# akloetgen/PARA-suite

Hardware: AMD Instinct MI355X
Metric: aligned reads/sec (10Mx50bp PAR-CLIP vs hg19-size genome) on MI355X; SAM bit-exact vs own CPU restatement (parity unpinned) (higher is better)
Workload: dtype u64

## Files before the change

### para-suite_amd/csrc/ps_kernels.hip

```cpp
#include <hip/hip_runtime.h>
#include <algorithm>
#include <cstdlib>
#include <stdexcept>
#include <string>
#include "ps_core.h"
#include "ps_narrow.h"
#include "ps_kernels.h"

namespace ps {

static const int PS_Q_CHUNK = 64;
#ifndef PS_BT_WAVES
#define PS_BT_WAVES 4
#endif

__device__ __forceinline__ unsigned long long wave_sum(unsigned long long v)
{
    for (int o = 32; o > 0; o >>= 1) v += __shfl_xor(v, o, 64);
    return v;
}
__device__ __forceinline__ void flush_stats(KStats *ks, const LaneStats &st)
{
    if (!ks) return;
    unsigned long long v[8] = {st.pairs, st.same, st.nodes, st.pushes, st.pops, st.lf, st.iters, st.exact};
// ... 100 lines not shown
        const unsigned long long wmask = __ballot(want), lmask = __ballot(L.mode != M_EXIT), hmask = __ballot(L.mode == M_HIT);
        if (lmask == 0) break;
        const bool stalled = (wmask | hmask) == lmask;
        const bool serve_hit = hmask != 0 && (__popcll(hmask) >= (int)hit_min || stalled);
        int fetch_r = -1;
        if (wmask) {
            const int cnt = __popcll(wmask);
            if (cnt >= (int)fetch_min || stalled) {
                const int rank = __popcll(wmask & lane_lt);
                int served = 0;
                while (served < cnt) {
                    if (q_next == q_end) {
                        if (exhausted) break;
                        unsigned int base = 0;
                        if (lane == 0) base = atomicAdd(queue, (unsigned int)PS_Q_CHUNK);
                        base = (unsigned int)__shfl((int)base, 0, 64);
                        if (base >= n_reads) { exhausted = true; break; }
                        q_next = (int)base;
                        q_end = (int)base + PS_Q_CHUNK < (int)n_reads ? (int)base + PS_Q_CHUNK : (int)n_reads;
                    }
                    const int take = q_end - q_next < cnt - served ? q_end - q_next : cnt - served;
                    if (want && rank >= served && rank < served + take) fetch_r = q_next + (rank - served);
                    q_next += take; served += take;
                }
                if (want && fetch_r < 0 && exhausted) fetch_r = (int)n_reads;
            }
        }
        bt_iter(a, h, L, m, fetch_r, serve_hit);
    }
    if (lane == 0) L.st.lf = (uint32_t)((wall_clock64() - t_start) >> 4);
    flush_stats(a.stats, L.st);
}


template <bool STATS, bool NB32>
__global__ void __launch_bounds__(256, PS_BT_WAVES) k_backtrack_n(const BtArgs *__restrict__ ap, BtHot hk, int lm_stride)
{
    const BtArgs &a = *ap;
    BtHot h; pin_hot(h, hk);
    uint32_t *const queue = reinterpret_cast<uint32_t *>(pin64(reinterpret_cast<unsigned long long>(a.queue)));
    const uint32_t n_reads = h.n_reads, fetch_min = pin32((uint32_t)a.fetch_min), hit_min = pin32((uint32_t)a.hit_min);
    extern __shared__ __attribute__((aligned(16))) uint8_t smem[];
    const int lane_g = blockIdx.x * blockDim.x + threadIdx.x;
    BtMem m;
    bt_mem_bind(m, smem + (size_t)threadIdx.x * lm_stride, h.len(), h.seed_len());
    uint8_t *const pool_private = reinterpret_cast<uint8_t *>(a.pool) + (size_t)lane_g * h.pool_cap * sizeof(Entry16);
    m.pool = pool_private;
    m.heads = nullptr;
    NLane L;
    nl_init(L);
    LaneStats st;
    ls_init(st);
    NtClock clk;
    for (int j = 0; j < 4; ++j) clk.tm[j] = 0;
    clk.t_last = 0;
#ifdef PS_STAMPS
    clk.t_last = __builtin_amdgcn_s_memtime();
#endif
    const int lane = threadIdx.x & 63;
    const unsigned long long t_start = STATS ? wall_clock64() : 0ull;
    uint32_t iters0 = 0;
    int q_next = 0, q_end = 0;
    bool exhausted = false;
    for (;;) {
        const int mode = nl_mode(L.ctl);
        const bool want = mode == M_FETCH;
        if (want && (L.ctl & NL_BIG)) {
            const unsigned int slot = (unsigned int)((reinterpret_cast<uint8_t *>(m.pool) - a.big_pool) / ((size_t)h.big_cap * sizeof(Entry16)));
            __threadfence();
            atomicExch(a.big_busy + slot, 0u);
            m.pool = pool_private;
            L.ctl &= ~NL_BIG;
        }
        const unsigned long long wmask = __ballot(want), lmask = __ballot(mode != M_EXIT), hmask = __ballot(mode == M_HIT);
        if (lmask == 0) break;
        const bool stalled = (wmask | hmask) == lmask;
        const bool serve_hit = hmask != 0 && (__popcll(hmask) >= (int)hit_min || stalled);
        int fetch_r = -1;
        if (wmask) {
            const int cnt = __popcll(wmask);
            if (cnt >= (int)fetch_min || stalled) {
                const int rank = (int)__builtin_amdgcn_mbcnt_hi((unsigned int)(wmask >> 32), __builtin_amdgcn_mbcnt_lo((unsigned int)wmask, 0u));
                int served = 0;
                while (served < cnt) {
                    if (q_next == q_end) {
                        if (exhausted) break;
                        unsigned int base = 0;
                        if (lane == 0) base = atomicAdd(queue, (unsigned int)PS_Q_CHUNK);
                        base = (unsigned int)__shfl((int)base, 0, 64);
                        if (base >= n_reads) { exhausted = true; break; }
                        q_next = (int)base;
                        q_end = (int)base + PS_Q_CHUNK < (int)n_reads ? (int)base + PS_Q_CHUNK : (int)n_reads;
                    }
                    const int take = q_end - q_next < cnt - served ? q_end - q_next : cnt - served;
                    if (want && rank >= served && rank < served + take) fetch_r = q_next + (rank - served);
                    q_next += take; served += take;
                }
                if (want && fetch_r < 0 && exhausted) fetch_r = (int)n_reads;
            }
        }
        unsigned long long gmask = __ballot(mode == M_GROW);
        while (gmask) {
            const int src = __ffsll((unsigned long long)gmask) - 1;
            gmask &= gmask - 1;
            const unsigned int n_big = a.n_big;
            unsigned int slot = n_big;
            if (lane == src) {
                unsigned int at = atomicAdd(a.big_next, 1u) % n_big;
                for (int tries = 0; tries < 256; ++tries) {
                    if (atomicCAS(a.big_busy + at, 0u, 1u) == 0u) { slot = at; break; }
                    at = at + 1u == n_big ? 0u : at + 1u;
                }
            }
            slot = (unsigned int)__shfl((int)slot, src, 64);
            const unsigned int n_copy = (unsigned int)__shfl((int)nl_bump(L), src, 64);
            const unsigned long long from = (unsigned long long)__shfl((long long)reinterpret_cast<unsigned long long>(m.pool), src, 64);
            if (slot < n_big) {
                const uint4 *sp = reinterpret_cast<const uint4 *>(from);
                uint4 *dp = reinterpret_cast<uint4 *>(a.big_pool + (size_t)slot * h.big_cap * sizeof(Entry16));
                for (unsigned int e = (unsigned int)lane; e < n_copy; e += 64u) dp[e] = sp[e];
                __threadfence();
                if (lane == src) { m.pool = dp; L.ctl = nl_set_mode(L.ctl | NL_BIG, M_EXPAND); }
            } else if (lane == src) L.ctl = nl_set_mode(nl_set_status(L.ctl, RS_OVERFLOW_POOL), M_POP);
        }
        nt_iter<STATS, NB32>(a, h, L, st, m, fetch_r, serve_hit, &clk);
        if (STATS && a.read_iters) {
            const int now = nl_mode(L.ctl);
            if (mode == M_FETCH && now != M_FETCH && now != M_EXIT) {
                iters0 = st.iters - 1u;
                const int len = nl_len(L), sl = h.seed_len();
                a.read_iters[PS_RI_WORDS * (size_t)L.r + 2] = (uint32_t)(m.cw[len - 1] & 0x7f) | ((h.use_seed() && sl > 0 && sl < len ? (uint32_t)(m.csw[sl - 1] & 0x7f) : 0u) << 8) | (a.est_ab ? (uint32_t)a.est_ab[L.r] << 16 : 0u);
                const uint32_t *cw32 = reinterpret_cast<const uint32_t *>(m.cw);
                for (int p = 0; p < 16; ++p) a.read_iters[PS_RI_WORDS * (size_t)L.r + 4 + p] = p < lm_ncw(len) ? cw32[p] : 0u;
            }
            if (mode != M_FETCH && mode != M_EXIT && now == M_FETCH) {
                uint32_t *ri = a.read_iters + PS_RI_WORDS * (size_t)L.r;
                ri[0] = st.iters - iters0; ri[1] = nl_bump(L);
                ri[3] = (uint32_t)nl_best_score(L) | ((uint32_t)nl_max_units(L) << 8) | ((uint32_t)nl_n_aln(L.ctl) << 16);
            }
        }
    }
    if (STATS) {
        if (lane == 0) st.lf = (uint32_t)((wall_clock64() - t_start) >> 4);
#ifdef PS_STAMPS
        st.nodes = lane == 0 ? (uint32_t)(clk.tm[0] >> 6) : 0; st.pushes = lane == 0 ? (uint32_t)(clk.tm[1] >> 6) : 0;
        st.pops = lane == 0 ? (uint32_t)(clk.tm[2] >> 6) : 0; st.exact = lane == 0 ? (uint32_t)(clk.tm[3] >> 6) : 0;
#endif
        flush_stats(a.stats, st);
    } else {
        st.nodes = st.pushes = st.pops = st.iters = st.exact = st.lf = 0;
        flush_stats(a.stats, st);
    }
}

__global__ void __launch_bounds__(256) k_sa2pos(IndexView ix, const bwtint *rows, bwtint *out, int n, KStats *stats)
{
    const int stride = gridDim.x * blockDim.x;
    int item = blockIdx.x * blockDim.x + threadIdx.x;
    LaneStats st = {0, 0, 0, 0, 0, 0, 0, 0};
    bool have = false; bwtint row = 0; uint32_t steps = 0;
    while (true) {
        if (!have) {
            if (item >= n) break;
            row = rows[item]; steps = 0; have = true;
        }
        if (!sa_walk_step(ix, row, steps, st)) {
            out[item] = (bwtint)steps + sa_sample(ix, row / (bwtint)ix.sa_intv);
            item += stride; have = false;
        }
    }
    flush_stats(stats, st);
}

__device__ __forceinline__ int text_sym(const IndexView &ix, bwtint p) { return p < ix.l_pac ? pac_base(ix.pac, p) : 3 - pac_base(ix.pac, 2 * ix.l_pac - 1 - p); }
__global__ void __launch_bounds__(256) k_index_check(IndexView ix, unsigned long long *out)
{
    unsigned long long rows = 0, bad_sym = 0, bad_sa = 0, longest = 0;
    const bwtint n_sa = ix.n_sa;
    for (bwtint t = (bwtint)blockIdx.x * blockDim.x + threadIdx.x; t < n_sa; t += (bwtint)gridDim.x * blockDim.x) {
        bwtint row = t * (bwtint)ix.sa_intv;
        bwtint p = t == 0 ? ix.seq_len : sa_sample(ix, t);
        unsigned long long steps = 0;
        do {
            if (p == 0) {
                if (row != ix.primary) ++bad_sym;
                row = 0; p = ix.seq_len;
            } else {
                if (row == ix.primary) { ++bad_sym; break; }
                int pos = 0;
                const uint32_t b = blk_of(row_to_stored(ix.primary, row), pos);
                Blk x;
                load_blk(ix.blocks, b, x);
                const int c = blk_sym(x, pos);
                if (c != text_sym(ix, p - 1)) ++bad_sym;
                row = L2_of(ix, c) + blk_count1(x, pos + 1, c);
                --p;
            }
// ... 23 lines not shown
    int32_t *E = H + (size_t)(a.len + 2) * 64;
    uint8_t *z = a.zbuf + (size_t)blockIdx.x * a.z_per_block + threadIdx.x;
    for (int it = blockIdx.x * 64 + threadIdx.x; it < a.n_items; it += gridDim.x * 64) {
        RefineItem q = a.items[it];
        const int qlen = a.lens ? a.lens[q.read] : a.len;
        int tlen = qlen + q.ref_shift;
        int d = tlen - qlen; if (d < 0) d = -d;
        int w = (int)(d * 1.5); if (w < 50) w = 50;
        const int r = q.read, len = qlen, n_reads = a.n_reads;
        const uint32_t *bases = a.bases, *nmask = a.nmask;
        const int strand = q.strand;
        uint32_t cig[PS_MAX_CIGAR];
        int n = banded_global(len,
            [&](int j) { int b = read_base(bases, nmask, n_reads, r, strand ? len - 1 - j : j); return b > 3 ? 4 : (strand ? 3 - b : b); },
            tlen, a.ix.pac, q.rb, w, H, E, 64, z, 64, cig, PS_MAX_CIGAR);
        a.n_cigar[it] = n;
        for (int j = 0; j < PS_MAX_CIGAR; ++j) a.cigar[(size_t)it * PS_MAX_CIGAR + j] = j < n ? cig[j] : 0;
    }
}

void launch_width(const WidthArgs &a, hipStream_t s)
{
    int blocks = (a.n_reads + 255) / 256;
    if (blocks > 256 * 8) blocks = 256 * 8;
    if (blocks < 1) blocks = 1;
    hipLaunchKernelGGL(k_width, dim3(a.use_seed ? 2 * blocks : blocks), dim3(256), 0, s, a);
}
__global__ void __launch_bounds__(256) k_jump_level(BtHot h, uint32_t *table, bwtint seq_len, int d)
{
    const uint32_t n = 1u << (2 * d);
    for (uint32_t s = blockIdx.x * blockDim.x + threadIdx.x; s < n; s += gridDim.x * blockDim.x) jump_fill_slot(h, table, seq_len, d, s);
}
void launch_jump_build(const IndexView &ix, uint32_t *table, int levels, hipStream_t s)
{
    BtArgs a{};
    a.ix = ix; a.ix.jump = nullptr; a.ix.jump_levels = 0;
    BtHot h;
    (void)bt_hot_make(a, h);
    for (int d = 0; d < levels; ++d) {
        const uint32_t n = 1u << (2 * d);
        const int blocks = (int)std::min<uint32_t>((n + 255u) / 256u, 256u * 16u);
        hipLaunchKernelGGL(k_jump_level, dim3(blocks), dim3(256), 0, s, h, table, ix.seq_len, d);
    }
}
bool launch_backtrack(const BtArgs &a_in, const BtArgs *d_args, BtArgs *h_stage, int n_blocks, int lm_stride, hipStream_t s, bool stats)
{
    BtArgs &a = *h_stage;
    a = a_in;
    const char *ej = std::getenv("PS_JUMP");
    const bool stats_plain = stats && !std::getenv("PS_STATS_JUMP");
    if (stats_plain || a.wide || (ej && std::atoi(ej) == 0)) { a.ix.jump = nullptr; a.ix.jump_levels = 0; }
    BtHot h;
    if (!bt_hot_make(a, h)) return false;
    (void)hipMemcpyAsync(const_cast<BtArgs *>(d_args), &a, sizeof(BtArgs), hipMemcpyHostToDevice, s);
    const size_t lds = (size_t)256 * lm_stride;
    const bool nb32 = a.md.n_buckets <= 32;
    typedef void (*KernelN)(const BtArgs *, BtHot, int);
    const KernelN kn = stats ? (nb32 ? k_backtrack_n<true, true> : k_backtrack_n<true, false>) : (nb32 ? k_backtrack_n<false, true> : k_backtrack_n<false, false>);
    const void *fn = a.wide ? reinterpret_cast<const void *>(k_backtrack_wide) : reinterpret_cast<const void *>(kn);
    set_dynamic_lds(fn, a.wide ? "k_backtrack_wide" : "k_backtrack_n", lds);
    if (a.wide) hipLaunchKernelGGL(k_backtrack_wide, dim3(n_blocks), dim3(256), lds, s, d_args, h, lm_stride);
    else hipLaunchKernelGGL(kn, dim3(n_blocks), dim3(256), lds, s, d_args, h, lm_stride);
    return true;
}
void launch_sa2pos(const IndexView &ix, const bwtint *rows, bwtint *out, int n, KStats *stats, hipStream_t s)
{
    int blocks = (n + 255) / 256;
    if (blocks > 256 * 8) blocks = 256 * 8;
    if (blocks < 1) blocks = 1;
    hipLaunchKernelGGL(k_sa2pos, dim3(blocks), dim3(256), 0, s, ix, rows, out, n, stats);
}
void launch_refine(const RefineArgs &a, int n_blocks, hipStream_t s)
{
    if (!a.hebuf || a.he_per_block < refine_he_words(a.len)) throw std::runtime_error("k_refine: H/E scratch missing or too small");
    hipLaunchKernelGGL(k_refine, dim3(n_blocks), dim3(64), 0, s, a);
}
void set_dynamic_lds(const void *kernel, const char *name, size_t bytes)
{
    if (bytes <= 48 * 1024) return;
    const std::string what = std::string(name) + ": " + std::to_string(bytes) + " B of dynamic LDS";
    if (bytes > PS_LDS_PER_CU) throw std::runtime_error(what + " requested, a CU has " + std::to_string(PS_LDS_PER_CU));
    const hipError_t e = hipFuncSetAttribute(kernel, hipFuncAttributeMaxDynamicSharedMemorySize, (int)bytes);
    if (e != hipSuccess) throw std::runtime_error(what + " refused: " + hipGetErrorString(e));
}

}
```

### para-suite_amd/csrc/ps_narrow.h

```cpp
#pragma once
#include "ps_core.h"

namespace ps {

PS_HD int nw_i(uint32_t wa) { return (int)(wa & 0xffu); }
PS_HD int nw_ldp(uint32_t wa) { return (int)((wa >> 8) & 0xffu); }
PS_HD int nw_mm(uint32_t wa) { return (int)((wa >> 16) & 0xffu); }
PS_HD int nw_state(uint32_t wa) { return (int)((wa >> 24) & 3u); }
PS_HD int nw_gapo(uint32_t wa) { return (int)((wa >> 26) & 7u); }
PS_HD int nw_gape(uint32_t wa) { return (int)(wa >> 29); }
PS_HD int nw_ins(uint32_t wb) { return (int)(wb & 7u); }
PS_HD int nw_del(uint32_t wb) { return (int)((wb >> 3) & 7u); }
PS_HD uint32_t nw_c(uint32_t wb) { return (wb >> 6) & 7u; }
PS_HD int nw_score(uint32_t wb) { return (int)((wb >> 9) & 0x7fu); }
static const uint32_t NW_KEEP = 0xFCFF0000u;
static const uint32_t NW_C_MASK = 7u << 6;
static const uint32_t NW_ROOT_C = 4u;

PS_HD int nl_mode(uint32_t ctl) { return (int)(ctl & 7u); }
PS_HD uint32_t nl_set_mode(uint32_t ctl, int mode) { return (ctl & ~7u) | (uint32_t)mode; }
static const uint32_t NL_HAVE_CUR = 8u, NL_STATUS = 7u << 4, NL_BIG = 1u << 7;
PS_HD int nl_status(uint32_t ctl) { return (int)((ctl >> 4) & 7u); }
PS_HD uint32_t nl_set_status(uint32_t ctl, int s) { return (ctl & ~NL_STATUS) | ((uint32_t)s << 4); }
PS_HD int nl_n_aln(uint32_t ctl) { return (int)(ctl >> 16); }

struct NLane {
    uint32_t kr, lr, wa, wb;
    uint32_t ctl;
    int r;
    uint32_t lim;
    uint32_t nsb;
    uint32_t n_phantom;
    uint32_t fh;
    uint32_t bm0, bm1;
    uint32_t rn0, rn1;
};
PS_HD int nl_best_score(const NLane &L) { return (int)(L.lim & 0xffu); }
PS_HD int nl_max_units(const NLane &L) { return (int)((L.lim >> 8) & 0xffu); }
PS_HD int nl_len(const NLane &L) { return (int)((L.lim >> 16) & 0xffu); }
PS_HD int nl_n_stack(const NLane &L) { return (int)(L.nsb & 0xffffu); }
PS_HD uint32_t nl_bump(const NLane &L) { return L.nsb >> 16; }
PS_HD uint32_t nl_phantom(const NLane &L) { return L.n_phantom & 0x00FFFFFFu; }
PS_HD int nl_est(const NLane &L) { return (int)(L.n_phantom >> 24); }

PS_HD void nl_init(NLane &L)
{
    L.kr = L.lr = L.wa = L.wb = 0; L.ctl = (uint32_t)M_FETCH; L.r = 0; L.lim = 0; L.nsb = 0;
    L.n_phantom = 0; L.fh = 0xffffu; L.bm0 = L.bm1 = 0; L.rn0 = L.rn1 = 0;
}
PS_HD void ls_init(LaneStats &st) { st.pairs = st.same = st.nodes = st.pushes = st.pops = st.iters = st.exact = st.lf = 0; }
PS_HD uint32_t ps_mul24(uint32_t x, uint32_t y)
{
#ifdef __HIP_DEVICE_COMPILE__
    return __umul24(x, y);
#else
    return x * y;
#endif
}

struct NtClock { unsigned long long tm[4]; unsigned long long t_last; };
#if defined(PS_STAMPS) && defined(__HIP_DEVICE_COMPILE__)
#define PS_USTAMP(clk, slot) do { if (STATS && (clk)) { const unsigned long long t_ = __builtin_amdgcn_s_memtime(); (clk)->tm[slot] += t_ - (clk)->t_last; (clk)->t_last = t_; } } while (0)
#else
#define PS_USTAMP(clk, slot) do { } while (0)
#endif

PS_HD bwtint nt_base(const BtHot &h, uint32_t c)
{
    return (bwtint)sel4s(h.L2lo[0], h.L2lo[1], h.L2lo[2], h.L2lo[3], (int)c) | ((bwtint)((h.L2hi >> c) & 1u) << 32);
}
PS_HD int nt_units(const BtHot &h, uint32_t wa, uint32_t wb)
{
    return h.profile() ? nw_score(wb) : nw_mm(wa) + nw_gapo(wa) + (h.mode_gape() ? nw_gape(wa) : 0);
}

PS_HD void blk_count4b(const Blk &b, int r, uint32_t cnt[4])
{
    uint32_t A = 0, B = 0, C = 0;
    const int q = r >> 5;
    const uint32_t part = (1u << (r & 31)) - 1u;
#pragma unroll
    for (int j = 0; j < 6; ++j) {
        const uint32_t m = j < q ? 0xFFFFFFFFu : (j == q ? part : 0u), lo = b.x[4 + j] & m, hi = b.x[10 + j] & m;
        A += ps_popc(lo); B += ps_popc(hi); C += ps_popc(lo & hi);
    }
    cnt[0] = b.x[0] + ((uint32_t)r - A - B + C);
    cnt[1] = b.x[1] + (A - C); cnt[2] = b.x[2] + (B - C); cnt[3] = b.x[3] + C;
}

#ifndef PS_OCC_COND
#define PS_OCC_COND 1
#endif
template <bool STATS>
PS_HD void nt_occ(const BtHot &h, uint32_t c, uint32_t kr, uint32_t lr, uint32_t ck[4], uint32_t cl[4], LaneStats &st)
{
    const bwtint base = nt_base(h, c);
    const bool need_k = c != NW_ROOT_C;
    int ol_ = 0, ok_ = 0;
    const uint32_t bl = blk_of(row_to_stored(h.primary, base + lr), ol_);
    uint32_t bk = blk_of(row_to_stored(h.primary, base + (bwtint)(need_k ? kr - 1u : 0u)), ok_);
    bk = need_k ? bk : 0u;
    const int rk = need_k ? ok_ + 1 : 0;
    Blk xl, xk;
    load_blk(h.blocks, bl, xl);
    if (PS_OCC_COND) {
        const bool other = bk != bl;
        if (other) load_blk(h.blocks, bk, xk);
        blk_count4b(xl, ol_ + 1, cl);
#pragma unroll
        for (int j = 0; j < 16; ++j) xk.x[j] = other ? xk.x[j] : xl.x[j];
    } else { load_blk(h.blocks, bk, xk); blk_count4b(xl, ol_ + 1, cl); }
    blk_count4b(xk, rk, ck);
    ++st.pairs; if (need_k && bk == bl) ++st.same;
// ... 218 lines not shown
        mode = M_POP;
    }
    if (mode == M_POP) {
        const int n_virtual = nl_n_stack(L) + ((L.ctl & NL_HAVE_CUR) ? 1 : 0);
        if (nl_phantom(L) && (long long)n_virtual + (long long)nl_phantom(L) > (long long)h.max_entries) {
            L.ctl = nl_set_status(L.ctl, RS_OVERFLOW_POOL); nt_finish_read(a, L); return 0;
        }
        if (n_virtual == 0 && nl_est(L) != 255 && nl_n_aln(L.ctl) == 0 && nl_status(L.ctl) == RS_OK) { NLane t = L; nt_restart_without_estimate(a, t, m); L = t; return 0; }
        if (n_virtual == 0 || n_virtual > (int)h.max_entries || nl_status(L.ctl) != RS_OK) { nt_finish_read(a, L); return 0; }
        if (L.ctl & NL_HAVE_CUR) L.ctl &= ~NL_HAVE_CUR;
        else { nt_pop<NB32>(L, m); if (STATS) ++st.pops; }
        L.ctl = nl_set_mode(L.ctl, M_POP);
        const int score = nw_score(L.wb), i1 = nw_i(L.wa);
        if (score > nl_best_score(L) + h.s_stop()) { nt_finish_read(a, L); return 0; }
        const int rem = nl_max_units(L) - nt_units(h, L.wa, L.wb);
        if (rem < 0) return 0;
        const int mleft = (int)(ps_mul24((uint32_t)rem, h.inv_c_min) >> 16);
        if (i1 > 0 && mleft < (int)(m.cw[i1 - 1] & 0x7f)) return 0;
        if (i1 == 0) { L.ctl = nl_set_mode(L.ctl, M_HIT); return 0; }
        const int st_ = nw_state(L.wa);
        mode = (mleft == 0 && (st_ == ST_M || h.mode_gape() || nw_gape(L.wa) == h.max_gape())) ? M_EXACT : M_EXPAND;
    }
    return mode;
}

struct NtStep { uint32_t ck[4], cl[4]; uint32_t cw_i, cw_im1, cs_i, cs_im1; int s, i; bool in_seed, tm, ctm; };

template <bool STATS>
PS_HD void nt_step_occ(const BtHot &h, NLane &L, LaneStats &st, BtMem &m, NtStep &q)
{
    const int len = nl_len(L), max_len = h.len();
    const int i = nw_i(L.wa) - 1;
    q.i = i;
    q.cw_i = m.cw[i]; q.cw_im1 = m.cw[i > 0 ? i - 1 : 0];
    const int ii = i - (len - h.seed_len());
    q.in_seed = h.use_seed() && len > h.seed_len() && ii > 0;
    q.cs_i = q.in_seed ? m.csw[ii] : 0u; q.cs_im1 = q.in_seed ? m.csw[ii - 1] : 0u;
    q.s = nt_seq_at(m, L, i, len, max_len);
    const int depth = nt_depth(len, L.wa, L.wb);
    q.tm = depth < (int)h.jump_levels; q.ctm = depth + 1 < (int)h.jump_levels;
    if (!q.tm) nt_occ<STATS>(h, nw_c(L.wb), L.kr, L.lr, q.ck, q.cl, st);
    else nt_jump(h, depth, L.kr, q.ck, q.cl);
}

template <bool STATS, bool NB32>
PS_HD void nt_tail(const BtHot &h, NLane &L, LaneStats &st, BtMem &m, const NtStep &q, int mode)
{
    const int len = nl_len(L), i = q.i, s = q.s;
    const uint32_t cw_i = q.cw_i, cw_im1 = q.cw_im1, cs_i = q.cs_i, cs_im1 = q.cs_im1;
    const bool in_seed = q.in_seed, tm = q.tm, ctm = q.ctm;
    uint32_t ck[4], cl[4];
#pragma unroll
    for (int c = 0; c < 4; ++c) { ck[c] = q.ck[c]; cl[c] = q.cl[c]; }
    if (mode == M_EXACT) {
        if (STATS) ++st.exact;
        L.ctl = nl_set_mode(L.ctl, M_POP);
        if (s > 3) return;
        const uint32_t ok = sel4(ck, s), ol = sel4(cl, s);
        if (ok >= ol) return;
        L.kr = ctm ? (L.kr << 2) | (uint32_t)s : ok + 1u; L.lr = ctm ? ol - ok : ol; L.wa -= 1u; L.wb = (L.wb & ~NW_C_MASK) | ((uint32_t)s << 6);
        L.ctl = nl_set_mode(L.ctl, i == 0 ? M_HIT : M_EXACT);
        return;
    }
    if (STATS) ++st.nodes;
    const uint32_t cap = (L.ctl & NL_BIG) ? h.big_cap : h.pool_cap;
    if (nl_bump(L) + 9u > cap) {
        if (!(L.ctl & NL_BIG) && h.has_big()) { L.ctl = nl_set_mode(L.ctl, M_GROW); return; }
        L.ctl = nl_set_mode(nl_set_status(L.ctl, cap >= 65535u ? RS_OVERFLOW_DEEP : RS_OVERFLOW_POOL), M_POP); return;
    }
    const int max_units = nl_max_units(L);
    const int e_un = nt_units(h, L.wa, L.wb), e_sc = nw_score(L.wb);
    const int rem = max_units - e_un;
    const uint32_t inv = h.inv_c_min;
    const int mleft = (int)(ps_mul24((uint32_t)rem, inv) >> 16);
    const int srem = h.seed_units() - e_un;
    const int m_seed = srem <= 0 ? 0 : (int)(ps_mul24((uint32_t)srem, inv) >> 16);
    bool allow_diff = true, allow_M = true;
    const int bnd_same = i > 0 ? (int)(cw_im1 & 0x7f) : 0;
    const int bnd_del = (int)(cw_i & 0x7f);
    if (i > 0) {
        if (bnd_same > mleft - 1) allow_diff = false;
        else if (bnd_same == mleft - 1 && bnd_del == mleft - 1 && (cw_i & 0x80u)) allow_M = false;
        if (in_seed) {
            const int s1 = (int)(cs_im1 & 0x7f), s0 = (int)(cs_i & 0x7f);
            if (s1 > m_seed - 1) allow_diff = false;
            else if (s1 == m_seed - 1 && s0 == m_seed - 1 && (cs_i & 0x80u)) allow_M = false;
        }
    }
    const int e_go = nw_gapo(L.wa), e_ge = nw_gape(L.wa), e_st = nw_state(L.wa);
    const int tmp = e_go + e_ge;
    const bool gap_ok = allow_diff && i >= h.indel_end_skip() + tmp && len - i >= h.indel_end_skip() + tmp;
    const bool from_m = e_st == ST_M, from_i = e_st == ST_I, from_d = e_st == ST_D;
    const uint32_t wa_keep = L.wa & NW_KEEP, pos2 = (uint32_t)i | ((uint32_t)i << 8);
    const uint32_t wb0 = L.wb & 0x1ffu;
    const uint32_t pkr = L.kr, plr = L.lr;
    const int need_same = (int)ps_mul24((uint32_t)bnd_same, h.c_min), need_del = (int)ps_mul24((uint32_t)bnd_del, h.c_min);
    const int cap_rem = nl_est(L) - e_sc, ut = h.u_tight();
    const int cap_same = cap_rem + (ut > need_same ? ut - need_same : 0), cap_del = cap_rem + (ut > need_del ? ut - need_del : 0);
    const int thr_same = (rem - need_same) < cap_same ? (rem - need_same) : cap_same, thr_del = (rem - need_del) < cap_del ? (rem - need_del) : cap_del;
    uint32_t phantom = 0, gmask = 0;
    int sc[9];
    uint32_t wa_i, wa_d;
    {
        const bool open = from_m && e_go < h.max_gapo(), ext = from_i && e_ge < h.max_gape();
        const int c = open ? h.u_gapo_ins() : h.u_gape();
        sc[0] = e_sc + (open ? h.s_gapo_ins() : h.s_gape());
        const bool cand = gap_ok && (open || ext) && c <= rem, go = cand && c <= thr_same;
        gmask |= go ? 1u : 0u;
        phantom += (cand && !go) ? 1u : 0u;
        wa_i = wa_keep + pos2 + ((uint32_t)ST_I << 24) + (open ? 1u << 26 : 1u << 29);
    }
    {
        const uint32_t occ = tm ? plr : plr - pkr + 1u;
        const bool open = from_m && e_go < h.max_gapo();
        const bool ext = from_d && e_ge < h.max_gape() && ((e_ge + e_go) * h.u_tight() < max_units || occ < (uint32_t)h.max_del_occ());
        const int c = open ? h.u_gapo_del() : h.u_gape();
        const int scd = e_sc + (open ? h.s_gapo_del() : h.s_gape());
        const bool cand = gap_ok && (open || ext) && c <= rem, go = cand && c <= thr_del;
        const uint32_t ne = (ck[0] < cl[0] ? 2u : 0u) | (ck[1] < cl[1] ? 4u : 0u) | (ck[2] < cl[2] ? 8u : 0u) | (ck[3] < cl[3] ? 16u : 0u);
        gmask |= go ? ne : 0u;
        if (cand && !go) phantom += ps_popc(ne);
        sc[1] = sc[2] = sc[3] = sc[4] = scd;
        wa_d = wa_keep + ((uint32_t)(i + 1) | ((uint32_t)(i + 1) << 8)) + ((uint32_t)ST_D << 24) + (open ? 1u << 26 : 1u << 29);
    }
    const bool do_mm = allow_diff && allow_M;
    const uint32_t s_word = cost_word(h.s_pk, s), u_word = h.profile() ? s_word : cost_word(h.u_pk, s);
    uint32_t xk[4], xl[4];
#pragma unroll
    for (int j = 1; j <= 4; ++j) {
        const int c = (s + j) & 3;
        xk[j - 1] = sel4(ck, c); xl[j - 1] = sel4(cl, c);
        sc[4 + j] = 0;
        if (j < 4 || s > 3) {
            const int cu = (int)((u_word >> (8 * c)) & 0xffu);
            sc[4 + j] = e_sc + (int)((s_word >> (8 * c)) & 0xffu);
            const bool cand = do_mm && xk[j - 1] < xl[j - 1] && cu <= rem, go = cand && cu <= thr_same;
            gmask |= go ? 1u << (4 + j) : 0u;
            phantom += (cand && !go) ? 1u : 0u;
        }
    }
    const uint32_t n_push = ps_popc(gmask), fr = L.fh;
    const bool reuse = fr != 0xffffu && n_push != 0u;
    const uint32_t slot0 = (L.nsb >> 16) - (reuse ? 1u : 0u);
    L.nsb += n_push + ((n_push - (reuse ? 1u : 0u)) << 16);
    L.fh = n_push ? 0xffffu : fr;
    if (STATS) st.pushes += n_push;
    uint32_t idx[9], raw[9];
#pragma unroll
    for (int j = 0; j < 9; ++j) {
        idx[j] = 0; raw[j] = 0;
        if ((gmask >> j) & 1u) {
            const uint32_t rank = ps_popc(gmask & ((1u << j) - 1u));
            idx[j] = (reuse && rank == 0u) ? fr : slot0 + rank;
            raw[j] = m.heads16[sc[j]];
            m.heads16[sc[j]] = (uint16_t)idx[j];
            if (NB32 || sc[j] < 32) L.bm0 |= 1u << sc[j]; else L.bm1 |= 1u << (sc[j] - 32);
        }
    }
#ifdef __HIP_DEVICE_COMPILE__
    asm volatile("" : "+v"(raw[0]), "+v"(raw[1]), "+v"(raw[2]), "+v"(raw[3]), "+v"(raw[4]), "+v"(raw[5]), "+v"(raw[6]), "+v"(raw[7]), "+v"(raw[8]));
#endif
    Entry16 *const pool = reinterpret_cast<Entry16 *>(m.pool);
#define NT_NEXT(j) (raw[j] << 16)
    if (gmask & 1u) { Entry16 e; e.k = pkr; e.l = plr; e.a = wa_i; e.b = (wb0 + 1u) | ((uint32_t)sc[0] << 9) | NT_NEXT(0); store16(pool + idx[0], e); }
    {
        const uint32_t wb_d = ((wb0 & 0x3fu) + (1u << 3)) | ((uint32_t)sc[1] << 9);
#pragma unroll
        for (int c = 0; c < 4; ++c)
            if ((gmask >> (1 + c)) & 1u) { Entry16 e; e.k = ctm ? (pkr << 2) | (uint32_t)c : ck[c] + 1u; e.l = ctm ? cl[c] - ck[c] : cl[c]; e.a = wa_d; e.b = wb_d | ((uint32_t)c << 6) | NT_NEXT(1 + c); store16(pool + idx[1 + c], e); }
    }
    {
        const uint32_t wa_x = wa_keep + pos2 + (1u << 16), wb_x = wb0 & 0x3fu;
#pragma unroll
        for (int j = 1; j <= 4; ++j) {
            const uint32_t c = (uint32_t)((s + j) & 3);
            if ((gmask >> (4 + j)) & 1u) { Entry16 e; e.k = ctm ? (pkr << 2) | c : xk[j - 1] + 1u; e.l = ctm ? xl[j - 1] - xk[j - 1] : xl[j - 1]; e.a = wa_x; e.b = wb_x | (c << 6) | ((uint32_t)sc[4 + j] << 9) | NT_NEXT(4 + j); store16(pool + idx[4 + j], e); }
        }
    }
#undef NT_NEXT
    L.ctl = nl_set_mode(L.ctl, M_POP);
    if (s < 4 && xk[3] < xl[3]) {
        L.kr = ctm ? (pkr << 2) | (uint32_t)s : xk[3] + 1u; L.lr = ctm ? xl[3] - xk[3] : xl[3]; L.wa = wa_keep + (uint32_t)i; L.wb = (L.wb & ~NW_C_MASK) | ((uint32_t)s << 6);
        L.ctl |= NL_HAVE_CUR;
    }
    L.n_phantom += phantom;
}

template <bool STATS, bool NB32>
PS_HD void nt_iter(const BtArgs &a, const BtHot &h, NLane &L, LaneStats &st, BtMem &m, int fetch_r, bool serve_hit, NtClock *clk = nullptr)
{
    PS_USTAMP(clk, 0);
    const int mode = nt_head<STATS, NB32>(a, h, L, st, m, fetch_r, serve_hit);
    PS_USTAMP(clk, 1);
    NtStep q;
    if (mode) nt_step_occ<STATS>(h, L, st, m, q);
#if defined(PS_STAMPS) && defined(__HIP_DEVICE_COMPILE__)
    if (STATS && clk && mode) asm volatile("" :: "v"(q.ck[0]), "v"(q.cl[0]), "v"(q.ck[3]), "v"(q.cl[3]));
#endif
    PS_USTAMP(clk, 2);
    if (mode) nt_tail<STATS, NB32>(h, L, st, m, q, mode);
    PS_USTAMP(clk, 3);
}

}
```

### para-suite_amd/csrc/ps_pipeline.hip

```cpp
#include <hip/hip_runtime.h>
#include <mutex>
#include <optional>
#include <hipcub/hipcub.hpp>
#include <algorithm>
#include <atomic>
#include <chrono>
#include <cmath>
#include <cstdio>
#include <cstring>
#include <functional>
#include <thread>
#include "ps_pipeline.h"
#include "ps_par.h"
#include "ps_core.h"

namespace ps {

typedef std::chrono::steady_clock Clock;
static double ms_since(Clock::time_point t0) { return std::chrono::duration<double, std::milli>(Clock::now() - t0).count(); }

void require_device(int device)
{
    int n = 0;
    hipError_t e = hipGetDeviceCount(&n);
// ... 319 lines not shown
                if (const char *e = std::getenv("PS_ORDER_SCALE")) em.log_scale = std::max(1, std::min(12, std::atoi(e)));
                if (d_lens) {
                    uint8_t *tab = wk->pin_get<uint8_t>("units_by_len_h2", 256);
                    for (int l2 = 0; l2 < 256; ++l2) { const int u = budget_diffs(ctx->opt, l2) * (ctx->opt.profile ? ctx->opt.unit : 1); tab[l2] = (uint8_t)(u > 255 ? 255 : u); }
                    uint8_t *d_tab = wk->ws_get<uint8_t>("units_by_len2", 256);
                    PS_HIP(hipMemcpyAsync(d_tab, tab, 256, hipMemcpyHostToDevice, s));
                    em.units_by_len = d_tab;
                }
                em.key = key; em.pred = nullptr;
                launch_effort_model(em, s);
            }
            launch_order_sort(key, n, wk->ws_get<uint32_t>("order_tmp", order_sort_tmp_words(n)), order, s);
            PS_HIP(hipGetLastError());
            t_order->mark();
            d_order = order; d_est = est;
        }
    }
    int dev_cus = 256;
    { hipDeviceProp_t p; if (hipGetDeviceProperties(&p, ctx->device) == hipSuccess && p.multiProcessorCount > 0) dev_cus = p.multiProcessorCount; }
    const int lm = lm_bytes(len, seed_len, md.n_buckets, wide);
    int per_cu = (int)((size_t)(160 * 1024) / ((size_t)256 * lm));
    if (per_cu < 1) throw Error("read length / score range too large for the per-lane LDS state");
    { const char *e = std::getenv("PS_MAX_PER_CU"); const int cap = e ? std::atoi(e) : 4; if (per_cu > cap) per_cu = cap; }
    int blocks = ctx->bt_blocks > 0 ? ctx->bt_blocks : dev_cus * per_cu;
    int need = (n + 255) / 256;
    if (blocks > need) blocks = need;
    const size_t per_lane = (size_t)pool_cap * (wide ? sizeof(Entry) : 16) + (wide ? PS_MAX_BUCKETS * 4 : 0);
    const size_t max_lanes = ((size_t)(wide ? 32 : 64) << 30) / per_lane;
    if ((size_t)blocks * 256 > max_lanes) blocks = (int)std::max<size_t>(1, max_lanes / 256);
    const int n_lanes = blocks * 256;
    uint8_t *pool = wk->ws_get<uint8_t>("pool", (size_t)n_lanes * pool_cap * (wide ? sizeof(Entry) : 16));
    uint32_t *heads = wide ? wk->ws_get<uint32_t>("heads", (size_t)n_lanes * PS_MAX_BUCKETS) : nullptr;
    uint32_t *queue = wk->ws_get<uint32_t>("queue", 16);
    PS_HIP(hipMemsetAsync(queue, 0, 64, s));
    BtArgs a; std::memset(&a, 0, sizeof a);
    a.ix = ctx->ix.view; a.md = md; a.n_reads = n; a.len = len; a.lens = d_lens; a.n_lanes = n_lanes;
    if (d_lens) {
        uint8_t *tab = wk->pin_get<uint8_t>("units_by_len_h", 256);
        for (int l2 = 0; l2 < 256; ++l2) { const int u = budget_diffs(ctx->opt, l2) * (ctx->opt.profile ? ctx->opt.unit : 1); tab[l2] = (uint8_t)(u > 255 ? 255 : u); }
        uint8_t *d_tab = wk->ws_get<uint8_t>("units_by_len", 256);
        PS_HIP(hipMemcpyAsync(d_tab, tab, 256, hipMemcpyHostToDevice, s));
        a.units_by_len = d_tab;
    }
    a.bases = d_bases; a.nmask = d_nmask; a.n_bw = (len + 15) / 16; a.n_mw = (len + 31) / 32;
    a.w = w; a.cwb = cwb; a.cswb = cswb;
    a.alns = alns; a.aln_cap = aln_cap; a.n_aln = n_aln; a.status = status;
    a.pool = pool; a.pool_cap = pool_cap; a.heads = heads; a.wide = wide ? 1 : 0; a.stats = b.d_stats.p + 1;
    a.queue = queue; a.fetch_min = ctx->fetch_min; a.hit_min = ctx->hit_min;
    a.order = d_order; a.est = d_est; a.est_ab = d_est_ab;
    a.cap_est = (first_tier && !wide && d_est && md.profile && !(std::getenv("PS_CAP") && std::atoi(std::getenv("PS_CAP")) == 0)) ? 1 : 0;
    if (a.cap_est) if (const char *e = std::getenv("PS_CAP_BIAS")) a.cap_est += std::max(0, std::min(200, std::atoi(e)));
    if (const char *e = std::getenv("PS_FETCH_MIN")) a.fetch_min = std::max(1, std::atoi(e));
    if (const char *e = std::getenv("PS_HIT_MIN")) a.hit_min = std::max(1, std::atoi(e));
    if (!wide && pool_cap < 65535 && ctx->n_big > 0) {
        a.big_cap = 65535; a.n_big = (uint32_t)std::min<int64_t>(ctx->n_big, std::max(64, n));
        a.big_pool = wk->ws_get<uint8_t>("big_pool", (size_t)a.n_big * a.big_cap * 16);
        a.big_next = queue + 4;
        a.big_busy = wk->ws_get<uint32_t>("big_busy", a.n_big);
        PS_HIP(hipMemsetAsync(a.big_busy, 0, (size_t)a.n_big * 4, s));
    }
    uint32_t *riters = nullptr;
    if (ctx->want_read_iters) { riters = wk->ws_get<uint32_t>("riters", (size_t)n * PS_RI_WORDS); PS_HIP(hipMemsetAsync(riters, 0, (size_t)n * PS_RI_WORDS * 4, s)); a.read_iters = riters; }
    { EvTimer t(s);
      if (!launch_backtrack(a, wk->ws_get<BtArgs>("btargs", 1), wk->pin_get<BtArgs>("btargs_h", 1), blocks, lm, s, ctx->want_kstats || ctx->want_read_iters)) throw Error("cost model outside the ranges the search kernel packs (gap/score fields must fit a byte)");
      PS_HIP(hipGetLastError());
      const double ms = t.stop(); b.tm.ms_backtrack += ms; ++b.tm.n_backtrack_launches;
      b.tm.ms_width += t_width->read();
      if (t_order) b.tm.ms_width += t_order->read();
      { double t0_ = 0, t1_ = 0; t.span(ctx->ref_event, t0_, t1_); if (b.tm.n_backtrack_launches == 1) b.tm.bt_begin_ms = t0_; b.tm.bt_end_ms = t1_; }
      if (std::getenv("PS_VERBOSE")) std::fprintf(stderr, "[parasuite-hip]   backtrack launch: %d reads x %d bp, stack %u%s, %d lanes, %.1f ms\n", n, len, pool_cap, wide ? " (wide)" : "", n_lanes, ms); }
    if (ctx->want_read_iters) { ctx->read_iters.resize((size_t)n * PS_RI_WORDS); PS_HIP(hipMemcpyAsync(ctx->read_iters.data(), riters, (size_t)n * PS_RI_WORDS * 4, hipMemcpyDeviceToHost, s)); PS_HIP(hipStreamSynchronize(s)); }
}

static void download_alns(Work *wk, int n, int aln_cap, const AlnRec *d_alns, const int32_t *d_n_aln,
                          std::vector<int32_t> &n_aln, std::vector<uint32_t> &off, std::vector<AlnRec> &alns)
{
    hipStream_t s = wk->stream;
    uint32_t *cnt = wk->ws_get<uint32_t>("cnt", n), *d_off = wk->ws_get<uint32_t>("off", (size_t)n + 1);
    hipLaunchKernelGGL(k_clip_counts, dim3((n + 255) / 256), dim3(256), 0, s, d_n_aln, aln_cap, n, cnt);
    size_t tb = 0;
    PS_HIP(hipcub::DeviceScan::ExclusiveSum(nullptr, tb, cnt, d_off, n, s));
    uint8_t *tmp = wk->ws_get<uint8_t>("scan_tmp", tb ? tb : 1);
    PS_HIP(hipcub::DeviceScan::ExclusiveSum(tmp, tb, cnt, d_off, n, s));
    int32_t *p_na = wk->pin_get<int32_t>("dl_n_aln", n); uint32_t *p_off = wk->pin_get<uint32_t>("dl_off", (size_t)n + 1);
    PS_HIP(hipMemcpyAsync(p_na, d_n_aln, (size_t)n * 4, hipMemcpyDeviceToHost, s));
    PS_HIP(hipMemcpyAsync(p_off, d_off, (size_t)n * 4, hipMemcpyDeviceToHost, s));
    PS_HIP(hipStreamSynchronize(s));
    uint32_t last = 0;
    if (n) { int m = p_na[n - 1]; last = p_off[n - 1] + (uint32_t)(m > aln_cap ? aln_cap : (m < 0 ? 0 : m)); }
    p_off[n] = last;
    n_aln.assign(p_na, p_na + n); off.assign(p_off, p_off + n + 1); alns.resize(last);
    if (last) {
        AlnRec *comp = wk->ws_get<AlnRec>("comp", last);
        hipLaunchKernelGGL(k_gather_alns, dim3((n + 255) / 256), dim3(256), 0, s, d_alns, aln_cap, d_n_aln, d_off, n, comp);
        AlnRec *p_al = wk->pin_get<AlnRec>("dl_alns", last);
        PS_HIP(hipMemcpyAsync(p_al, comp, (size_t)last * sizeof(AlnRec), hipMemcpyDeviceToHost, s));
        PS_HIP(hipStreamSynchronize(s));
        std::memcpy(alns.data(), p_al, (size_t)last * sizeof(AlnRec));
    }
}

__global__ void k_classify(const AlnRec *alns, int aln_cap, const int32_t *n_aln, const uint8_t *status, const int32_t *ids,
                           int n, int n_occ, uint8_t *cls_out)
{
    for (int r = blockIdx.x * blockDim.x + threadIdx.x; r < n; r += gridDim.x * blockDim.x) {
        uint8_t c = 0;
// ... 639 lines not shown
```

### para-suite_amd/csrc/ps_types.h

```cpp
#pragma once
#include <stdint.h>
#include <stddef.h>

#ifdef __HIPCC__
#define PS_HD __host__ __device__ __forceinline__
#define PS_COLD __host__ __device__ inline __attribute__((noinline))
#else
#define PS_HD inline
#define PS_COLD inline
#endif

namespace ps {

typedef uint64_t bwtint;
static const bwtint PS_MAX_ROWS = (1ull << 33) - 64;

static const int PS_BLK_SYMS = 192;
struct OccBlock { uint32_t cnt[4]; uint32_t sym[12]; };

struct IndexView {
    const OccBlock *blocks;
    const uint32_t *sa;
    const uint32_t *sa_hi;
    const uint8_t  *pac;
// ... 11 lines not shown
    uint8_t u_mm[5][4], s_mm[5][4];
    uint32_t u_mm_pk[5], s_mm_pk[5];
    int32_t u_gapo_ins, s_gapo_ins, u_gapo_del, s_gapo_del, u_gape, s_gape;
    int32_t s_stop, u_tight, c_min, inv_c_min , max_units, n_buckets;
    int32_t max_gapo, max_gape, mode_gape, indel_end_skip, max_del_occ, max_entries;
    int32_t seed_len, max_seed_diff, max_top2, use_seed, len, profile;
};
static const int PS_MAX_BUCKETS = 128;
static const int PS_MAX_LEN = 250;

struct Entry {
    bwtint k, l;
    uint16_t score, units;
    uint8_t i, last_diff_pos, n_mm, n_gapo, n_gape, n_ins, n_del, state;
    uint32_t next;
};
static const uint32_t PS_NIL = 0xFFFFFFFFu;
enum { ST_M = 0, ST_I = 1, ST_D = 2 };

struct AlnRec {
    bwtint k, l;
    uint16_t score, units;
    uint8_t n_mm, n_gapo, n_gape, n_ins, n_del, pad[7];
};

enum { RS_OK = 0, RS_OVERFLOW_POOL = 1, RS_OVERFLOW_ALN = 2, RS_BAD_SCORE = 3,
       RS_OVERFLOW_DEEP = 4 };

struct KStats {
    unsigned long long occ_pairs, occ_same_blk, nodes, pushes, pops, lf_steps, iters, exact_steps;
};

static const int PS_RI_WORDS = 20;
struct BtArgs {
    IndexView ix;
    Model md;
    int n_reads, len, n_lanes;
    const int32_t *lens;
    const uint8_t *units_by_len;
    const uint32_t *bases; const uint32_t *nmask; int n_bw, n_mw;
    uint32_t *w; const uint32_t *cwb; const uint32_t *cswb;
    AlnRec *alns; int aln_cap; int32_t *n_aln; uint8_t *status;
    void *pool; uint32_t pool_cap;
    uint32_t *heads;
    int wide;
    uint8_t *big_pool; uint32_t big_cap, n_big; uint32_t *big_busy; uint32_t *big_next;
    uint32_t *queue;
    const int32_t *order;
    const uint8_t *est; const uint16_t *est_ab;
    int cap_est;
    uint32_t *read_iters;
    int hit_min;
    int fetch_min;
    KStats *stats;
};

}
```

Measured before the change: 9.003 million.

## Amortize wave-level scheduling service across iterations and reorder node expansion

The per-iteration wave service (big-pool release, fetch ballot, queue refill, grow handling) now runs only every N iterations, default 4, via a phase counter. Skipped iterations fall back to servicing immediately if no lane can make progress or a lane needs grow or release. The big-pool slot index is computed with a reciprocal multiply instead of a 64-bit divide. Node expansion is reordered to compute candidate values before the EXACT and full-pool early exits, with an asm barrier to schedule loads early. Fetching reads and serving hits less often can leave lanes idle longer in exchange for less ballot and atomic overhead.

```diff
diff --git a/para-suite_amd/csrc/ps_kernels.hip b/para-suite_amd/csrc/ps_kernels.hip
--- a/para-suite_amd/csrc/ps_kernels.hip
+++ b/para-suite_amd/csrc/ps_kernels.hip
@@ -176,7 +176,7 @@
     LaneStats st;
     ls_init(st);
     NtClock clk;
-    for (int j = 0; j < 4; ++j) clk.tm[j] = 0;
+    for (int j = 0; j < 6; ++j) clk.tm[j] = 0;
     clk.t_last = 0;
 #ifdef PS_STAMPS
     clk.t_last = __builtin_amdgcn_s_memtime();
@@ -186,68 +186,83 @@
     uint32_t iters0 = 0;
     int q_next = 0, q_end = 0;
     bool exhausted = false;
+    const uint32_t service_every = pin32((uint32_t)(a.service_every > 1 ? a.service_every : 1));
+    uint32_t phase = 0;
     for (;;) {
         const int mode = nl_mode(L.ctl);
-        const bool want = mode == M_FETCH;
-        if (want && (L.ctl & NL_BIG)) {
-            const unsigned int slot = (unsigned int)((reinterpret_cast<uint8_t *>(m.pool) - a.big_pool) / ((size_t)h.big_cap * sizeof(Entry16)));
-            __threadfence();
-            atomicExch(a.big_busy + slot, 0u);
-            m.pool = pool_private;
-            L.ctl &= ~NL_BIG;
-        }
-        const unsigned long long wmask = __ballot(want), lmask = __ballot(mode != M_EXIT), hmask = __ballot(mode == M_HIT);
-        if (lmask == 0) break;
-        const bool stalled = (wmask | hmask) == lmask;
-        const bool serve_hit = hmask != 0 && (__popcll(hmask) >= (int)hit_min || stalled);
         int fetch_r = -1;
-        if (wmask) {
-            const int cnt = __popcll(wmask);
-            if (cnt >= (int)fetch_min || stalled) {
-                const int rank = (int)__builtin_amdgcn_mbcnt_hi((unsigned int)(wmask >> 32), __builtin_amdgcn_mbcnt_lo((unsigned int)wmask, 0u));
-                int served = 0;
-                while (served < cnt) {
-                    if (q_next == q_end) {
-                        if (exhausted) break;
-                        unsigned int base = 0;
-                        if (lane == 0) base = atomicAdd(queue, (unsigned int)PS_Q_CHUNK);
-                        base = (unsigned int)__shfl((int)base, 0, 64);
-                        if (base >= n_reads) { exhausted = true; break; }
-                        q_next = (int)base;
-                        q_end = (int)base + PS_Q_CHUNK < (int)n_reads ? (int)base + PS_Q_CHUNK : (int)n_reads;
+        bool serve_hit = false;
+#ifdef PS_STAMPS
+        const unsigned long long t_iter = clk.t_last;
+#endif
+        if (phase == 0) {
+            const bool want = mode == M_FETCH;
+            if (want && (L.ctl & NL_BIG)) {
+                const unsigned int slot = nt_big_slot((uint32_t)((size_t)(reinterpret_cast<uint8_t *>(m.pool) - a.big_pool) / sizeof(Entry16)), a.big_rcp);
+                __threadfence();
+                atomicExch(a.big_busy + slot, 0u);
+                m.pool = pool_private;
+                L.ctl &= ~NL_BIG;
+            }
+            const unsigned long long wmask = __ballot(want), lmask = __ballot(mode != M_EXIT), hmask = __ballot(mode == M_HIT);
+            if (lmask == 0) break;
+            const bool stalled = (wmask | hmask) == lmask;
+            serve_hit = hmask != 0 && (__popcll(hmask) >= (int)hit_min || stalled);
+            if (wmask) {
+                const int cnt = __popcll(wmask);
+                if (cnt >= (int)fetch_min || stalled) {
+                    const int rank = (int)__builtin_amdgcn_mbcnt_hi((unsigned int)(wmask >> 32), __builtin_amdgcn_mbcnt_lo((unsigned int)wmask, 0u));
+                    int served = 0;
+                    while (served < cnt) {
+                        if (q_next == q_end) {
+                            if (exhausted) break;
+                            unsigned int base = 0;
+                            if (lane == 0) base = atomicAdd(queue, (unsigned int)PS_Q_CHUNK);
+                            base = (unsigned int)__shfl((int)base, 0, 64);
+                            if (base >= n_reads) { exhausted = true; break; }
+                            q_next = (int)base;
+                            q_end = (int)base + PS_Q_CHUNK < (int)n_reads ? (int)base + PS_Q_CHUNK : (int)n_reads;
+                        }
+                        const int take = q_end - q_next < cnt - served ? q_end - q_next : cnt - served;
+                        if (want && rank >= served && rank < served + take) fetch_r = q_next + (rank - served);
+                        q_next += take; served += take;
                     }
-                    const int take = q_end - q_next < cnt - served ? q_end - q_next : cnt - served;
-                    if (want && rank >= served && rank < served + take) fetch_r = q_next + (rank - served);
-                    q_next += take; served += take;
+                    if (want && fetch_r < 0 && exhausted) fetch_r = (int)n_reads;
                 }
-                if (want && fetch_r < 0 && exhausted) fetch_r = (int)n_reads;
-            }
-        }
-        unsigned long long gmask = __ballot(mode == M_GROW);
-        while (gmask) {
-            const int src = __ffsll((unsigned long long)gmask) - 1;
-            gmask &= gmask - 1;
-            const unsigned int n_big = a.n_big;
-            unsigned int slot = n_big;
-            if (lane == src) {
-                unsigned int at = atomicAdd(a.big_next, 1u) % n_big;
-                for (int tries = 0; tries < 256; ++tries) {
-                    if (atomicCAS(a.big_busy + at, 0u, 1u) == 0u) { slot = at; break; }
-                    at = at + 1u == n_big ? 0u : at + 1u;
+            }
+            unsigned long long gmask = __ballot(mode == M_GROW);
+            while (gmask) {
+                const int src = __ffsll((unsigned long long)gmask) - 1;
+                gmask &= gmask - 1;
+                const unsigned int n_big = a.n_big;
+                unsigned int slot = n_big;
+                if (lane == src) {
+                    unsigned int at = atomicAdd(a.big_next, 1u) % n_big;
+                    for (int tries = 0; tries < 256; ++tries) {
+                        if (atomicCAS(a.big_busy + at, 0u, 1u) == 0u) { slot = at; break; }
+                        at = at + 1u == n_big ? 0u : at + 1u;
+                    }
                 }
-            }
-            slot = (unsigned int)__shfl((int)slot, src, 64);
-            const unsigned int n_copy = (unsigned int)__shfl((int)nl_bump(L), src, 64);
-            const unsigned long long from = (unsigned long long)__shfl((long long)reinterpret_cast<unsigned long long>(m.pool), src, 64);
-            if (slot < n_big) {
-                const uint4 *sp = reinterpret_cast<const uint4 *>(from);
-                uint4 *dp = reinterpret_cast<uint4 *>(a.big_pool + (size_t)slot * h.big_cap * sizeof(Entry16));
-                for (unsigned int e = (unsigned int)lane; e < n_copy; e += 64u) dp[e] = sp[e];
-                __threadfence();
-                if (lane == src) { m.pool = dp; L.ctl = nl_set_mode(L.ctl | NL_BIG, M_EXPAND); }
-            } else if (lane == src) L.ctl = nl_set_mode(nl_set_status(L.ctl, RS_OVERFLOW_POOL), M_POP);
+                slot = (unsigned int)__shfl((int)slot, src, 64);
+                const unsigned int n_copy = (unsigned int)__shfl((int)nl_bump(L), src, 64);
+                const unsigned long long from = (unsigned long long)__shfl((long long)reinterpret_cast<unsigned long long>(m.pool), src, 64);
+                if (slot < n_big) {
+                    const uint4 *sp = reinterpret_cast<const uint4 *>(from);
+                    uint4 *dp = reinterpret_cast<uint4 *>(a.big_pool + (size_t)slot * h.big_cap * sizeof(Entry16));
+                    for (unsigned int e = (unsigned int)lane; e < n_copy; e += 64u) dp[e] = sp[e];
+                    __threadfence();
+                    if (lane == src) { m.pool = dp; L.ctl = nl_set_mode(L.ctl | NL_BIG, M_EXPAND); }
+                } else if (lane == src) L.ctl = nl_set_mode(nl_set_status(L.ctl, RS_OVERFLOW_POOL), M_POP);
+            }
+        } else if (__ballot(mode == M_POP || mode == M_EXACT || mode == M_EXPAND) == 0 || __ballot(mode == M_GROW || (mode == M_FETCH && (L.ctl & NL_BIG))) != 0) {
+            phase = 0;
+            continue;
         }
         nt_iter<STATS, NB32>(a, h, L, st, m, fetch_r, serve_hit, &clk);
+#ifdef PS_STAMPS
+        if (phase == 0) clk.tm[5] += clk.t_last - t_iter;
+#endif
+        phase = phase + 1u >= service_every ? 0u : phase + 1u;
         if (STATS && a.read_iters) {
             const int now = nl_mode(L.ctl);
             if (mode == M_FETCH && now != M_FETCH && now != M_EXIT) {
@@ -267,6 +282,7 @@
     if (STATS) {
         if (lane == 0) st.lf = (uint32_t)((wall_clock64() - t_start) >> 4);
 #ifdef PS_STAMPS
+        st.pairs = lane == 0 ? (uint32_t)(clk.tm[4] >> 6) : 0; st.same = lane == 0 ? (uint32_t)(clk.tm[5] >> 6) : 0;
         st.nodes = lane == 0 ? (uint32_t)(clk.tm[0] >> 6) : 0; st.pushes = lane == 0 ? (uint32_t)(clk.tm[1] >> 6) : 0;
         st.pops = lane == 0 ? (uint32_t)(clk.tm[2] >> 6) : 0; st.exact = lane == 0 ? (uint32_t)(clk.tm[3] >> 6) : 0;
 #endif
@@ -396,6 +412,10 @@
     if (stats_plain || a.wide || (ej && std::atoi(ej) == 0)) { a.ix.jump = nullptr; a.ix.jump_levels = 0; }
     BtHot h;
     if (!bt_hot_make(a, h)) return false;
+    if (a.big_cap) {
+        if ((unsigned long long)a.n_big * a.big_cap > 0xFFFFFFFFull) return false;
+        a.big_rcp = nt_big_rcp(a.big_cap);
+    }
     (void)hipMemcpyAsync(const_cast<BtArgs *>(d_args), &a, sizeof(BtArgs), hipMemcpyHostToDevice, s);
     const size_t lds = (size_t)256 * lm_stride;
     const bool nb32 = a.md.n_buckets <= 32;
diff --git a/para-suite_amd/csrc/ps_narrow.h b/para-suite_amd/csrc/ps_narrow.h
--- a/para-suite_amd/csrc/ps_narrow.h
+++ b/para-suite_amd/csrc/ps_narrow.h
@@ -58,7 +58,10 @@
 #endif
 }
 
-struct NtClock { unsigned long long tm[4]; unsigned long long t_last; };
+PS_HD uint32_t nt_big_rcp(uint32_t big_cap) { return (uint32_t)(0x100000000ull / big_cap) + 1u; }
+PS_HD uint32_t nt_big_slot(uint32_t first_entry, uint32_t rcp) { return (uint32_t)(((unsigned long long)first_entry * rcp) >> 32); }
+
+struct NtClock { unsigned long long tm[6]; unsigned long long t_last; };
 #if defined(PS_STAMPS) && defined(__HIP_DEVICE_COMPILE__)
 #define PS_USTAMP(clk, slot) do { if (STATS && (clk)) { const unsigned long long t_ = __builtin_amdgcn_s_memtime(); (clk)->tm[slot] += t_ - (clk)->t_last; (clk)->t_last = t_; } } while (0)
 #else
@@ -383,22 +386,8 @@
     uint32_t ck[4], cl[4];
 #pragma unroll
     for (int c = 0; c < 4; ++c) { ck[c] = q.ck[c]; cl[c] = q.cl[c]; }
-    if (mode == M_EXACT) {
-        if (STATS) ++st.exact;
-        L.ctl = nl_set_mode(L.ctl, M_POP);
-        if (s > 3) return;
-        const uint32_t ok = sel4(ck, s), ol = sel4(cl, s);
-        if (ok >= ol) return;
-        L.kr = ctm ? (L.kr << 2) | (uint32_t)s : ok + 1u; L.lr = ctm ? ol - ok : ol; L.wa -= 1u; L.wb = (L.wb & ~NW_C_MASK) | ((uint32_t)s << 6);
-        L.ctl = nl_set_mode(L.ctl, i == 0 ? M_HIT : M_EXACT);
-        return;
-    }
-    if (STATS) ++st.nodes;
     const uint32_t cap = (L.ctl & NL_BIG) ? h.big_cap : h.pool_cap;
-    if (nl_bump(L) + 9u > cap) {
-        if (!(L.ctl & NL_BIG) && h.has_big()) { L.ctl = nl_set_mode(L.ctl, M_GROW); return; }
-        L.ctl = nl_set_mode(nl_set_status(L.ctl, cap >= 65535u ? RS_OVERFLOW_DEEP : RS_OVERFLOW_POOL), M_POP); return;
-    }
+    const bool full = nl_bump(L) + 9u > cap;
     const int max_units = nl_max_units(L);
     const int e_un = nt_units(h, L.wa, L.wb), e_sc = nw_score(L.wb);
     const int rem = max_units - e_un;
@@ -432,6 +421,7 @@
     uint32_t phantom = 0, gmask = 0;
     int sc[9];
     uint32_t wa_i, wa_d;
+    bool cand_d, go_d;
     {
         const bool open = from_m && e_go < h.max_gapo(), ext = from_i && e_ge < h.max_gape();
         const int c = open ? h.u_gapo_ins() : h.u_gape();
@@ -447,15 +437,40 @@
         const bool ext = from_d && e_ge < h.max_gape() && ((e_ge + e_go) * h.u_tight() < max_units || occ < (uint32_t)h.max_del_occ());
         const int c = open ? h.u_gapo_del() : h.u_gape();
         const int scd = e_sc + (open ? h.s_gapo_del() : h.s_gape());
-        const bool cand = gap_ok && (open || ext) && c <= rem, go = cand && c <= thr_del;
-        const uint32_t ne = (ck[0] < cl[0] ? 2u : 0u) | (ck[1] < cl[1] ? 4u : 0u) | (ck[2] < cl[2] ? 8u : 0u) | (ck[3] < cl[3] ? 16u : 0u);
-        gmask |= go ? ne : 0u;
-        if (cand && !go) phantom += ps_popc(ne);
+        cand_d = gap_ok && (open || ext) && c <= rem; go_d = cand_d && c <= thr_del;
         sc[1] = sc[2] = sc[3] = sc[4] = scd;
         wa_d = wa_keep + ((uint32_t)(i + 1) | ((uint32_t)(i + 1) << 8)) + ((uint32_t)ST_D << 24) + (open ? 1u << 26 : 1u << 29);
     }
     const bool do_mm = allow_diff && allow_M;
     const uint32_t s_word = cost_word(h.s_pk, s), u_word = h.profile() ? s_word : cost_word(h.u_pk, s);
+#ifdef __HIP_DEVICE_COMPILE__
+    {
+        uint32_t f_ = (gap_ok ? 1u : 0u) | (do_mm ? 2u : 0u) | (cand_d ? 4u : 0u) | (go_d ? 8u : 0u) | (full ? 16u : 0u);
+        asm volatile("" :: "v"(ck[0]), "v"(ck[1]), "v"(ck[2]), "v"(ck[3]), "v"(cl[0]), "v"(cl[1]), "v"(cl[2]), "v"(cl[3]), "v"(f_), "v"(gmask), "v"(phantom),
+                     "v"(thr_same), "v"(rem), "v"(sc[0]), "v"(sc[1]), "v"(wa_i), "v"(wa_d), "v"(s_word), "v"(u_word));
+        (void)f_;
+    }
+#endif
+    if (mode == M_EXACT) {
+        if (STATS) ++st.exact;
+        L.ctl = nl_set_mode(L.ctl, M_POP);
+        if (s > 3) return;
+        const uint32_t ok = sel4(ck, s), ol = sel4(cl, s);
+        if (ok >= ol) return;
+        L.kr = ctm ? (L.kr << 2) | (uint32_t)s : ok + 1u; L.lr = ctm ? ol - ok : ol; L.wa -= 1u; L.wb = (L.wb & ~NW_C_MASK) | ((uint32_t)s << 6);
+        L.ctl = nl_set_mode(L.ctl, i == 0 ? M_HIT : M_EXACT);
+        return;
+    }
+    if (STATS) ++st.nodes;
+    if (full) {
+        if (!(L.ctl & NL_BIG) && h.has_big()) { L.ctl = nl_set_mode(L.ctl, M_GROW); return; }
+        L.ctl = nl_set_mode(nl_set_status(L.ctl, cap >= 65535u ? RS_OVERFLOW_DEEP : RS_OVERFLOW_POOL), M_POP); return;
+    }
+    {
+        const uint32_t ne = (ck[0] < cl[0] ? 2u : 0u) | (ck[1] < cl[1] ? 4u : 0u) | (ck[2] < cl[2] ? 8u : 0u) | (ck[3] < cl[3] ? 16u : 0u);
+        gmask |= go_d ? ne : 0u;
+        if (cand_d && !go_d) phantom += ps_popc(ne);
+    }
     uint32_t xk[4], xl[4];
 #pragma unroll
     for (int j = 1; j <= 4; ++j) {
@@ -531,6 +546,10 @@
     PS_USTAMP(clk, 2);
     if (mode) nt_tail<STATS, NB32>(h, L, st, m, q, mode);
     PS_USTAMP(clk, 3);
-}
-
-}
+#if defined(PS_STAMPS) && defined(PS_STAMPS_WAIT) && defined(__HIP_DEVICE_COMPILE__)
+    if (STATS && clk) asm volatile("s_waitcnt vmcnt(0)" ::: "memory");
+#endif
+    PS_USTAMP(clk, 4);
+}
+
+}
diff --git a/para-suite_amd/csrc/ps_pipeline.hip b/para-suite_amd/csrc/ps_pipeline.hip
--- a/para-suite_amd/csrc/ps_pipeline.hip
+++ b/para-suite_amd/csrc/ps_pipeline.hip
@@ -395,6 +395,7 @@
     if (a.cap_est) if (const char *e = std::getenv("PS_CAP_BIAS")) a.cap_est += std::max(0, std::min(200, std::atoi(e)));
     if (const char *e = std::getenv("PS_FETCH_MIN")) a.fetch_min = std::max(1, std::atoi(e));
     if (const char *e = std::getenv("PS_HIT_MIN")) a.hit_min = std::max(1, std::atoi(e));
+    { const char *e = std::getenv("PS_SERVICE_EVERY"); a.service_every = e ? std::max(1, std::min(64, std::atoi(e))) : 4; }
     if (!wide && pool_cap < 65535 && ctx->n_big > 0) {
         a.big_cap = 65535; a.n_big = (uint32_t)std::min<int64_t>(ctx->n_big, std::max(64, n));
         a.big_pool = wk->ws_get<uint8_t>("big_pool", (size_t)a.n_big * a.big_cap * 16);
diff --git a/para-suite_amd/csrc/ps_types.h b/para-suite_amd/csrc/ps_types.h
--- a/para-suite_amd/csrc/ps_types.h
+++ b/para-suite_amd/csrc/ps_types.h
@@ -87,6 +87,8 @@
     uint32_t *read_iters;
     int hit_min;
     int fetch_min;
+    int service_every;
+    uint32_t big_rcp;
     KStats *stats;
 };
 
```

Result: no change. 8.952 million (-0.6%).
